# balazs-bamer/cdpr-simulation

Measured on AMD Instinct MI355X. Metric: CDPR sim-steps/sec (whole node), 65 536 parallel 8-cable robots, 1 ms dt, higher is better.
Workload: dtype f32

## Files before the change

### cdpr-simulation_amd/csrc/cdpr_onestep_kernel.hpp

```cpp
#pragma once
#include "cdpr_step_kernel.hpp"

namespace cdpr {

CDPR_DEV void row_to_lds(const float4* src, float4* dst_row) {
  __builtin_amdgcn_global_load_lds((const __attribute__((address_space(1))) void*)src, (__attribute__((address_space(3))) void*)dst_row, 16, 0, 0);
}


template <int NP, bool PR = false>
CDPR_DEV void pid_pairs(const StepArgs& a, int calls, bool is_vel, const v2f (&desired)[NP], const v2f (&actual)[NP], const v2f (&win)[NP][kWin],
                        v2f (&ierr)[NP], v2f (&f)[NP], v2f (&e_new)[NP], float& dbg_p, float& dbg_i, float& dbg_d, bool is_force = false) {
  const PidCoef c = pid_coef<PR>(a, is_vel);
  const bool run = (!PR || calls != 0) && !is_force;
  const bool full = calls >= c.nbuf;
  const float (&wt)[kWin + 2] = a.wrow;
  v2f error[NP], acc[NP];
#pragma unroll
  for (int k = 0; k < NP; ++k) {
    error[k] = desired[k] - actual[k];
    acc[k] = splat(wt[kWin]) * error[k];
  }
#pragma unroll
  for (int j = 0; j < kWin; ++j) {
// ... 260 lines not shown
  }

  if (PERSIST && more) {
    const uint32_t noff = nrr * 16u;
    if (run_pid) {
#pragma unroll
      for (int j = 0; j < kCtrl; ++j)
        row_to_lds(reinterpret_cast<const float4*>(reinterpret_cast<const char*>(a.state + (size_t)(P + j) * st) + noff), &stage[j][0]);
      if (kCmdLds) {
        const float* ncp = a.cmd + (size_t)nrr * N;
#pragma unroll
        for (int g = 0; g < kCmdRows; ++g) row_to_lds(reinterpret_cast<const float4*>(ncp) + g, &stage[kCtrl + g][0]);
      }
    }
  }

  CDPR_STAMP(5);
  v2f applied[NP];
  int td_flag = 0;
  if (TD) {
    v2f df[NP];
#pragma unroll
    for (int k = 0; k < NP; ++k) df[k] = f[k] - splat(a.td_mid);
    float g[6];
    if (FK) {
      jt_times<NP>(jest, df, g);
      normal_solve<NP, false>(jest, 0.f, g);
    } else {
      jt_times<NP>(jac, df, g);
      normal_solve<NP, false>(jac, 0.f, g);
    }
#pragma unroll
    for (int k = 0; k < NP; ++k) {
      v2f t = splat(a.td_mid);
#pragma unroll
      for (int c = 0; c < 6; ++c) t = fma2(g[c], FK ? jest[k][c] : jac[k][c], t);
      const v2f tc = max2(min2(t, splat(a.td_max)), splat(a.td_min));
      td_flag |= (tc.x != t.x) ? 1 : 0;
      if (2 * k + 1 < N) td_flag |= (tc.y != t.y) ? 1 : 0;
      applied[k] = tc;
    }
  } else {
#pragma unroll
    for (int k = 0; k < NP; ++k) applied[k] = f[k];
  }
  if (a.vel_limit > 0.f) {
#pragma unroll
    for (int k = 0; k < NP; ++k) {
      applied[k].x = (qd[k].x > a.vel_limit && applied[k].x > 0.f) || (qd[k].x < -a.vel_limit && applied[k].x < 0.f) ? 0.f : applied[k].x;
      applied[k].y = (qd[k].y > a.vel_limit && applied[k].y > 0.f) || (qd[k].y < -a.vel_limit && applied[k].y < 0.f) ? 0.f : applied[k].y;
    }
  }
  if (a.effort >= 0.f) {
#pragma unroll
    for (int k = 0; k < NP; ++k) applied[k] = max2(min2(applied[k], splat(a.effort)), splat(-a.effort));
  }

  if (a.dbg && live) {
    float* d = a.dbg + (size_t)r * 9;
    if (dbg_wrote) {
      d[0] = dbg_p;
      d[1] = dbg_i;
      d[2] = dbg_d;
      d[3] = desired[0].x;
    }
    d[4] = applied[0].x;
  }
  if (publish && live) {
    store_slot(a.obs, st, 3, woff, make_float4(s.wz, fk_res, (float)fk_it, pack_flags(td_flag, travel_mask<N>(a, q))));
#pragma unroll
    for (int g = 0; g < G; ++g) {
      const int k0 = 2 * g, k1 = (2 * g + 1 < NP) ? 2 * g + 1 : 2 * g;
      const bool has = (2 * g + 1 < NP);
      store_slot(a.obs, st, 4 + 2 * G + g, woff,
                make_float4(applied[k0].x, applied[k0].y, has ? applied[k1].x : 0.f, has ? applied[k1].y : 0.f));
    }
  }

  CDPR_STAMP(6);
  {
    v2f tens[NP];
#pragma unroll
    for (int k = 0; k < NP; ++k) {
      tens[k] = fma2(-a.damping, qd[k], applied[k]);
      if (a.unilateral) tens[k] = max2(tens[k], splat(0.f));
    }
    if (FK) {
      uint32_t again = 0;
      asm volatile("" : "+v"(again));
      v2f len2[NP], l02[NP];
      ik_pairs<N, false>(lds + again, s.px, s.py, s.pz, s.qx, s.qy, s.qz, s.qw, len2, jac, l02);
    }
    float w[6];
    jt_times<NP>(jac, tens, w);
    w[0] = a.fgx - w[0];
    w[1] = a.fgy - w[1];
    w[2] = a.fgz - w[2];
    w[3] = -w[3];
    w[4] = -w[4];
    w[5] = -w[5];
    integrate(a, s, w);
  }
  if (PERSIST && more) {
    constexpr int kDmaOps = kCtrl + kCmdRows;
    static_assert(kDmaOps < 64, "vmcnt is a 6-bit counter");
    if (run_pid)
      __builtin_amdgcn_s_waitcnt(vmcnt_imm(kDmaOps));
    else
      __builtin_amdgcn_s_waitcnt(vmcnt_imm(0));
    asm volatile("" : "+a"(n0), "+a"(n1), "+a"(n2), "+a"(n3), "+a"(n4));
  }
  if (live) {
    CDPR_STORE_STATE(a.state, st, 0, woff, make_float4(s.px, s.py, s.pz, s.qx));
    CDPR_STORE_STATE(a.state, st, 1, woff, make_float4(s.qy, s.qz, s.qw, s.vx));
    CDPR_STORE_STATE(a.state, st, 2, woff, make_float4(s.vy, s.vz, s.wx, s.wy));
    CDPR_STORE_STATE(a.state, st, 3, woff, make_float4(s.wz, fkx, fky, fkz));
    if (FK) CDPR_STORE_STATE(a.state, st, 4, woff, make_float4(fkqx, fkqy, fkqz, fkqw));
  }
  CDPR_STAMP(7);
  if (!(PERSIST && more)) break;
  blk = nblk;
  r = nr;
  rr = nrr;
  live = r < a.batch;
  off = rr * 16u, woff = r * 16u;
  p0 = make_float4(n0.x, n0.y, n0.z, n0.w), p1 = make_float4(n1.x, n1.y, n1.z, n1.w), p2 = make_float4(n2.x, n2.y, n2.z, n2.w);
  p3 = make_float4(n3.x, n3.y, n3.z, n3.w), p4 = make_float4(n4.x, n4.y, n4.z, n4.w);
  staged = run_pid;
  }
}

#ifndef CDPR_CTL_LOAD_DELAY
#define CDPR_CTL_LOAD_DELAY 8
#endif
#ifndef CDPR_SPLIT_PRIO
#define CDPR_SPLIT_PRIO 1
#endif
#ifdef CDPR_STAMPS
#define CDPR_SPLIT_STAMP(i)                                                                                          \
  do {                                                                                                               \
    __builtin_amdgcn_sched_barrier(0);                                                                               \
    if (a.stamps && lane == 0) a.stamps[(size_t)blockIdx.x * 8 + (i)] = __builtin_amdgcn_s_memrealtime();           \
    __builtin_amdgcn_sched_barrier(0);                                                                               \
  } while (0)
#else
#define CDPR_SPLIT_STAMP(i) do { } while (0)
#endif
#if defined(CDPR_STAMPS) && defined(CDPR_STAMPS_ITER)
#define CDPR_CTL_STAMP(i) do { } while (0)
#else
#define CDPR_CTL_STAMP(i) CDPR_SPLIT_STAMP(i)
#endif

template <int N, int XS, int ES, bool RAISED = true>
CDPR_DEV void split_estimator_wave(const StepArgs& a, float* geo, float gval, uint32_t lane, bool live, size_t st, uint32_t off, uint32_t woff,
                                   const float4& p0, const float4& p1, const float4& p3, const v2f* x_force, v2f* x_tension, float* x_est) {
  constexpr int NP = cable_pairs(N);
#if defined(CDPR_STAMPS) && defined(CDPR_STAMPS_CLOCK)
  const unsigned long long clk0 = __builtin_amdgcn_s_memtime();
#endif
#if CDPR_SPLIT_PRIO == 1 || CDPR_SPLIT_PRIO == 4
  if (RAISED) __builtin_amdgcn_s_setprio(3);
#elif CDPR_SPLIT_PRIO == 3 || CDPR_SPLIT_PRIO == 5
  if (RAISED) __builtin_amdgcn_s_setprio(2);
#endif
  const float4 p4 = load_slot(a.state, st, 4, off);
  if (lane < NP * kGeomFloatsPerPair) geo[lane] = gval;
  __builtin_amdgcn_fence(__ATOMIC_RELEASE, "wavefront");
  __builtin_amdgcn_wave_barrier();
  __builtin_amdgcn_fence(__ATOMIC_ACQUIRE, "wavefront");
  float fkx = p3.y, fky = p3.z, fkz = p3.w, fkqx = p4.x, fkqy = p4.y, fkqz = p4.z, fkqw = p4.w;
  v2f len[NP];
  {
    v2f jac[NP][6], l0[NP];
    ik_pairs<N, false>(geo, p0.x, p0.y, p0.z, p0.w, p1.x, p1.y, p1.z, len, jac, l0);
  }
  float fk_res = 0.f;
  int fk_it = 0;
  v2f jest[NP][6];
  {
    v2f elen[NP], unused[NP];
    bool active = true;
    for (int it = 0; it < a.fk_iters; ++it) {
      ik_pairs<N, false>(geo, fkx, fky, fkz, fkqx, fkqy, fkqz, fkqw, elen, jest, unused);
      v2f res[NP];
      v2f rm = splat(0.f);
#pragma unroll
      for (int k = 0; k < NP; ++k) {
        res[k] = len[k] - elen[k];
        rm = max2(rm, abs2(res[k]));
      }
      active = active && !(fmaxf(rm.x, rm.y) < a.fk_tol);
      float g[6];
      jt_times<NP>(jest, res, g);
      normal_solve<NP>(jest, a.fk_lambda, g);
      if (active) {
        fkx += g[0];
        fky += g[1];
        fkz += g[2];
        quat_apply_rotvec(fkqx, fkqy, fkqz, fkqw, g[3], g[4], g[5]);
        ++fk_it;
      }
#ifdef CDPR_STAMPS_ITER
      if (it < 3) {
        asm volatile("" ::"v"(fkqw));
        __builtin_amdgcn_sched_barrier(0);
        if (a.stamps && lane == 0) a.stamps[(size_t)blockIdx.x * 8 + 4 + it] = __builtin_amdgcn_s_memrealtime();
        __builtin_amdgcn_sched_barrier(0);
      }
#endif
    }
    ik_pairs<N, false>(geo, fkx, fky, fkz, fkqx, fkqy, fkqz, fkqw, elen, jest, unused);
    v2f rm = splat(0.f);
#pragma unroll
    for (int k = 0; k < NP; ++k) rm = max2(rm, abs2(len[k] - elen[k]));
    fk_res = fmaxf(rm.x, rm.y);
  }
  if (live) store_slot_aux<CDPR_SPLIT_PLAT_AUX>(a.state, st, 4, woff, make_float4(fkqx, fkqy, fkqz, fkqw));
  CDPR_SPLIT_STAMP(1);
  v2f td_l[6][3];
  float td_invd[6];
  normal_matrix_pk<NP, false>(jest, 0.f, td_l);
  chol_factor_pk(td_l, td_invd);
  __builtin_amdgcn_s_waitcnt(0xC07F);
  __builtin_amdgcn_s_barrier();
  CDPR_SPLIT_STAMP(2);
  __builtin_amdgcn_fence(__ATOMIC_ACQUIRE, "workgroup");
  v2f f[NP], df[NP], t_out[NP];
#pragma unroll
  for (int k = 0; k < NP; ++k) {
    f[k] = x_force[k * XS + lane];
    df[k] = f[k] - splat(a.td_mid);
  }
  int td_flag = 0;
  {
    float g[6];
    jt_times<NP>(jest, df, g);
    chol_apply_pk(td_l, td_invd, g);
#pragma unroll
    for (int k = 0; k < NP; ++k) {
      v2f t = splat(a.td_mid);
#pragma unroll
      for (int c = 0; c < 6; ++c) t = fma2(g[c], jest[k][c], t);
      const v2f tc = max2(min2(t, splat(a.td_max)), splat(a.td_min));
      td_flag |= (tc.x != t.x) ? 1 : 0;
      if (2 * k + 1 < N) td_flag |= (tc.y != t.y) ? 1 : 0;
      t_out[k] = tc;
    }
  }
#pragma unroll
  for (int k = 0; k < NP; ++k) x_tension[k * XS + lane] = t_out[k];
  x_est[0 * ES + lane] = fkx;
  x_est[1 * ES + lane] = fky;
  x_est[2 * ES + lane] = fkz;
  x_est[3 * ES + lane] = fk_res;
  x_est[4 * ES + lane] = (float)fk_it;
  x_est[5 * ES + lane] = (float)td_flag;
  __builtin_amdgcn_fence(__ATOMIC_RELEASE, "workgroup");
  __builtin_amdgcn_s_waitcnt(0xC07F);
  CDPR_SPLIT_STAMP(3);
#if defined(CDPR_STAMPS) && defined(CDPR_STAMPS_CLOCK)
  if (a.stamps && lane == 0) a.stamps[(size_t)blockIdx.x * 8 + 7] = __builtin_amdgcn_s_memtime() - clk0;
#endif
  __builtin_amdgcn_s_barrier();
}

template <int N, bool PR = false>
__global__ __launch_bounds__(128, 2) void cdpr_split_kernel(const StepArgs a) {
  constexpr int NP = cable_pairs(N);
  constexpr int P = plat_slots(true);
  constexpr int G = joint_groups(N);
  constexpr int NH = (NP + 1) / 2;
  __shared__ __attribute__((aligned(16))) float lds[2][NP * kGeomFloatsPerPair];
  __shared__ v2f x_force[NP][64];
  __shared__ v2f x_tension[NP][64];
  __shared__ float x_est[6][64];

  const uint32_t swap = __builtin_popcount(blockIdx.x & a.split_swap) & 1u;
  const uint32_t wave = (threadIdx.x >> 6) ^ swap, lane = threadIdx.x & 63u;
  const uint32_t r = blockIdx.x * 64u + lane;
  const uint32_t rr = (r < a.batch) ? r : (a.batch - 1u);
  const bool live = r < a.batch;
  const size_t st = a.stride;
  const uint32_t off = rr * 16u, woff = r * 16u;
  float* const geo = lds[wave];

  if (wave == 0) CDPR_SPLIT_STAMP(0);
#ifdef CDPR_STAMPS
  if (a.stamps && lane == 0)
    reinterpret_cast<uint32_t*>(&a.stamps[(size_t)blockIdx.x * 8 + 7])[threadIdx.x >> 6] =
        (__builtin_amdgcn_s_getreg((16 - 1) << 11 | 4) & 0xffffu) | ((__builtin_amdgcn_s_getreg((4 - 1) << 11 | 20) & 0xfu) << 16);
#endif
  const float gval = (lane < NP * kGeomFloatsPerPair) ? a.geom[lane] : 0.f;
  const float4 p0 = load_slot(a.state, st, 0, off), p1 = load_slot(a.state, st, 1, off), p2 = load_slot(a.state, st, 2, off),
               p3 = load_slot(a.state, st, 3, off);
  if (wave == 0) {
    split_estimator_wave<N, 64, 64>(a, geo, gval, lane, live, st, off, woff, p0, p1, p3, &x_force[0][0], &x_tension[0][0], &x_est[0][0]);
    return;
  }
#if CDPR_SPLIT_PRIO == 2 || CDPR_SPLIT_PRIO == 5
  __builtin_amdgcn_s_setprio(3);
#endif
#if CDPR_CTL_LOAD_DELAY > 0
  __builtin_amdgcn_s_sleep(CDPR_CTL_LOAD_DELAY);
#endif
  constexpr int kCtrl = 5 * NP + NH;
  float4 wraw[NP][5], hraw[NH];
#pragma unroll
  for (int k = 0; k < NP; ++k) {
#pragma unroll
    for (int m = 0; m < 5; ++m) wraw[k][m] = load_slot(a.state, st, P + 5 * k + m, off);
  }
#pragma unroll
  for (int g = 0; g < NH; ++g) hraw[g] = load_slot(a.state, st, P + 5 * NP + g, off);
  (void)kCtrl;
  v2f desired[NP];
#pragma unroll
  for (int k = 0; k < NP; ++k) desired[k] = splat(0.f);
  const float* cp = a.cmd + (size_t)rr * N;
  if (N % 4 == 0) {
#pragma unroll
    for (int g = 0; g < N / 4; ++g) {
      const float4 v = reinterpret_cast<const float4*>(cp)[g];
      desired[2 * g] = (v2f){v.x, v.y};
      desired[2 * g + 1] = (v2f){v.z, v.w};
    }
  } else {
#pragma unroll
    for (int i = 0; i < N; ++i) {
      if (i & 1)
        desired[i / 2].y = cp[i];
      else
        desired[i / 2].x = cp[i];
    }
  }
  if (lane < NP * kGeomFloatsPerPair) geo[lane] = gval;
  __builtin_amdgcn_fence(__ATOMIC_RELEASE, "wavefront");
  __builtin_amdgcn_wave_barrier();
  __builtin_amdgcn_fence(__ATOMIC_ACQUIRE, "wavefront");

  Platform s;
  s.px = p0.x; s.py = p0.y; s.pz = p0.z; s.qx = p0.w;
  s.qy = p1.x; s.qz = p1.y; s.qw = p1.z; s.vx = p1.w;
  s.vy = p2.x; s.vz = p2.y; s.wx = p2.z; s.wy = p2.w;
  s.wz = p3.x;

  v2f len[NP], q[NP], qd[NP], jac[NP][6];
  {
    v2f l0[NP];
    ik_pairs<N, true>(geo, s.px, s.py, s.pz, s.qx, s.qy, s.qz, s.qw, len, jac, l0);
#pragma unroll
    for (int k = 0; k < NP; ++k) {
      q[k] = l0[k] - len[k];
      qd[k] = -fma2(s.wz, jac[k][5], fma2(s.wy, jac[k][4], fma2(s.wx, jac[k][3],
                    fma2(s.vz, jac[k][2], fma2(s.vy, jac[k][1], splat(s.vx) * jac[k][0])))));
    }
  }
  const bool publish = (a.publish_mask & 1ull) != 0ull;
  if (publish && live) {
    store_slot(a.obs, st, 0, woff, make_float4(s.px, s.py, s.pz, s.qx));
    store_slot(a.obs, st, 1, woff, make_float4(s.qy, s.qz, s.qw, s.vx));
    store_slot(a.obs, st, 2, woff, make_float4(s.vy, s.vz, s.wx, s.wy));
#pragma unroll
    for (int g = 0; g < G; ++g) {
      const int k0 = 2 * g, k1 = (2 * g + 1 < NP) ? 2 * g + 1 : 2 * g;
      const bool has = (2 * g + 1 < NP);
      store_slot(a.obs, st, 4 + g, woff, make_float4(q[k0].x, q[k0].y, has ? q[k1].x : 0.f, has ? q[k1].y : 0.f));
      store_slot(a.obs, st, 4 + G + g, woff, make_float4(qd[k0].x, qd[k0].y, has ? qd[k1].x : 0.f, has ? qd[k1].y : 0.f));
    }
  }

  v2f f[NP], e_new[NP], ierr[NP];
#pragma unroll
  for (int k = 0; k < NP; ++k) {
    f[k] = splat(0.f);
    e_new[k] = splat(0.f);
    ierr[k] = (k & 1) ? (v2f){hraw[k / 2].z, hraw[k / 2].w} : (v2f){hraw[k / 2].x, hraw[k / 2].y};
  }
  float dbg_p = 0.f, dbg_i = 0.f, dbg_d = 0.f;
  bool dbg_wrote = false;
  const bool first_world = (a.flags & kFlagFirstWorldStep) != 0u;
  uint32_t meta = 0u;
  if (PR) meta = a.meta[rr];
  const int calls = PR ? (int)(meta >> kMetaCallShift) : a.pid_calls;
  if (PR && live && !first_world) a.meta[r] = (uint8_t)((meta & kMetaModeMask) | ((uint32_t)min(calls + 1, (int)kMetaCallMax) << kMetaCallShift));
  const bool force_mode = !PR && (a.flags & kFlagForceMode) != 0u;
  if (force_mode && !first_world) {
#pragma unroll
    for (int k = 0; k < NP; ++k) f[k] = desired[k];
  } else if (!first_world && (PR || calls != 0)) {
    v2f win[NP][kWin];
#pragma unroll
    for (int k = 0; k < NP; ++k) {
#pragma unroll
      for (int m = 0; m < 5; ++m) {
        win[k][2 * m] = (v2f){wraw[k][m].x, wraw[k][m].y};
        win[k][2 * m + 1] = (v2f){wraw[k][m].z, wraw[k][m].w};
      }
    }
    const bool actual_is_vel = PR ? ((meta & kMetaModeMask) == kMetaVelocity) : ((a.flags & kFlagActualIsVelocity) != 0u);
    v2f actual[NP];
#pragma unroll
    for (int k = 0; k < NP; ++k) actual[k] = actual_is_vel ? qd[k] : q[k];
    const int ring_slot = a.ring_slot;
    const bool is_force = PR && (meta & kMetaModeMask) == kMetaForce;
#if CDPR_SPLIT_PRIO == 3 || CDPR_SPLIT_PRIO == 4
    __builtin_amdgcn_s_setprio(3);
#endif
    pid_pairs<NP, PR>(a, calls, actual_is_vel, desired, actual, win, ierr, f, e_new, dbg_p, dbg_i, dbg_d, is_force);
    dbg_wrote = (!PR || calls != 0) && !is_force;
    if (live) {
#pragma unroll
      for (int m = 0; m < 5; ++m) {
        if (m == (ring_slot >> 1)) {
#pragma unroll
          for (int k = 0; k < NP; ++k) CDPR_STORE_STATE(a.state, st, P + 5 * k + m, woff, ring_row(win[k], m, e_new[k], ring_slot));
        }
      }
#pragma unroll
      for (int g = 0; g < NH; ++g) {
        const int k1 = (2 * g + 1 < NP) ? 2 * g + 1 : 2 * g;
        CDPR_STORE_STATE(a.state, st, P + 5 * NP + g, woff, make_float4(ierr[2 * g].x, ierr[2 * g].y, ierr[k1].x, ierr[k1].y));
      }
    }
  }
#pragma unroll
  for (int k = 0; k < NP; ++k) x_force[k][lane] = f[k];
  __builtin_amdgcn_fence(__ATOMIC_RELEASE, "workgroup");
  __builtin_amdgcn_s_waitcnt(0xC07F);
  CDPR_CTL_STAMP(4);
#if CDPR_SPLIT_PRIO >= 3
  __builtin_amdgcn_s_setprio(0);
#endif
  __builtin_amdgcn_s_barrier();
  __builtin_amdgcn_s_barrier();
  CDPR_CTL_STAMP(5);
  __builtin_amdgcn_fence(__ATOMIC_ACQUIRE, "workgroup");
  v2f applied[NP];
#pragma unroll
  for (int k = 0; k < NP; ++k) applied[k] = x_tension[k][lane];
  const float fkx = x_est[0][lane], fky = x_est[1][lane], fkz = x_est[2][lane], fk_res = x_est[3][lane], fk_it = x_est[4][lane],
              td_flag = x_est[5][lane];
  if (a.vel_limit > 0.f) {
#pragma unroll
    for (int k = 0; k < NP; ++k) {
      applied[k].x = (qd[k].x > a.vel_limit && applied[k].x > 0.f) || (qd[k].x < -a.vel_limit && applied[k].x < 0.f) ? 0.f : applied[k].x;
      applied[k].y = (qd[k].y > a.vel_limit && applied[k].y > 0.f) || (qd[k].y < -a.vel_limit && applied[k].y < 0.f) ? 0.f : applied[k].y;
    }
  }
  if (a.effort >= 0.f) {
#pragma unroll
    for (int k = 0; k < NP; ++k) applied[k] = max2(min2(applied[k], splat(a.effort)), splat(-a.effort));
  }
  if (a.dbg && live) {
    float* d = a.dbg + (size_t)r * 9;
    if (dbg_wrote) {
      d[0] = dbg_p;
      d[1] = dbg_i;
      d[2] = dbg_d;
      d[3] = desired[0].x;
    }
    d[4] = applied[0].x;
  }
  if (publish && live) {
    store_slot(a.obs, st, 3, woff, make_float4(s.wz, fk_res, fk_it, a.travel_on ? pack_flags((int)td_flag, travel_mask<N>(a, q)) : td_flag));
#pragma unroll
    for (int g = 0; g < G; ++g) {
      const int k0 = 2 * g, k1 = (2 * g + 1 < NP) ? 2 * g + 1 : 2 * g;
      const bool has = (2 * g + 1 < NP);
      store_slot(a.obs, st, 4 + 2 * G + g, woff,
                 make_float4(applied[k0].x, applied[k0].y, has ? applied[k1].x : 0.f, has ? applied[k1].y : 0.f));
    }
  }
  {
    v2f tens[NP];
#pragma unroll
    for (int k = 0; k < NP; ++k) {
      tens[k] = fma2(-a.damping, qd[k], applied[k]);
      if (a.unilateral) tens[k] = max2(tens[k], splat(0.f));
    }
    float w[6];
    jt_times<NP>(jac, tens, w);
    w[0] = a.fgx - w[0];
    w[1] = a.fgy - w[1];
    w[2] = a.fgz - w[2];
    w[3] = -w[3];
    w[4] = -w[4];
    w[5] = -w[5];
    integrate(a, s, w);
  }
  if (live) {
    store_slot_aux<CDPR_SPLIT_PLAT_AUX>(a.state, st, 0, woff, make_float4(s.px, s.py, s.pz, s.qx));
    store_slot_aux<CDPR_SPLIT_PLAT_AUX>(a.state, st, 1, woff, make_float4(s.qy, s.qz, s.qw, s.vx));
    store_slot_aux<CDPR_SPLIT_PLAT_AUX>(a.state, st, 2, woff, make_float4(s.vy, s.vz, s.wx, s.wy));
    store_slot_aux<CDPR_SPLIT_PLAT_AUX>(a.state, st, 3, woff, make_float4(s.wz, fkx, fky, fkz));
  }
  CDPR_CTL_STAMP(6);
}

}
```

### cdpr-simulation_amd/csrc/cdpr_step_kernel.hpp

```cpp
#pragma once
#include <hip/hip_runtime.h>
#include <stdint.h>

namespace cdpr {

constexpr int kMaxCables = 8;
constexpr int kWin = 10;
constexpr int kGeomFloatsPerPair = 16;

typedef float v2f __attribute__((ext_vector_type(2)));

enum StepFlags : uint32_t {
  kFlagFirstWorldStep = 1u << 0,
  kFlagRolloutResetPid = 1u << 1,
  kFlagActualIsVelocity = 1u << 2,
  kFlagPublishAll = 1u << 4,
  kFlagForceMode = 1u << 3,
};

struct PidSet {
  float kf, kp, ki, kd, inv_ki, imax, imin, cmax, cmin;
  int clamp_cmd;
};

// ... 234 lines not shown
    for (int i = j + 1; i < 6; ++i) {
      float s = m[i][j];
#pragma unroll
      for (int k = 0; k < j; ++k) s = fmaf(-m[i][k], m[j][k], s);
      m[i][j] = s * invd[j];
    }
  }
#pragma unroll
  for (int i = 0; i < 6; ++i) {
    float s = g[i];
#pragma unroll
    for (int k = 0; k < i; ++k) s = fmaf(-m[i][k], g[k], s);
    g[i] = s * invd[i];
  }
#pragma unroll
  for (int i = 5; i >= 0; --i) {
    float s = g[i];
#pragma unroll
    for (int k = i + 1; k < 6; ++k) s = fmaf(-m[k][i], g[k], s);
    g[i] = s * invd[i];
  }
}

#ifndef CDPR_CHOL_PACKED
#define CDPR_CHOL_PACKED 1
#endif

CDPR_DEV void chol_factor_pk(v2f (&mp)[6][3], float (&invd)[6]) {
#pragma unroll
  for (int j = 0; j < 6; ++j) {
    const int p0 = j / 2;
    invd[j] = __frsqrt_rn((j & 1) ? mp[j][p0].y : mp[j][p0].x);
#pragma unroll
    for (int p = p0; p < 3; ++p) mp[j][p] = mp[j][p] * splat(invd[j]);
#pragma unroll
    for (int c = j + 1; c < 6; ++c) {
      const float lcj = (c & 1) ? mp[j][c / 2].y : mp[j][c / 2].x;
#pragma unroll
      for (int p = c / 2; p < 3; ++p) mp[c][p] = fma2(-lcj, mp[j][p], mp[c][p]);
    }
  }
}

CDPR_DEV void chol_apply_pk(const v2f (&mp)[6][3], const float (&invd)[6], float (&g)[6]) {
  v2f gp[3] = {(v2f){g[0], g[1]}, (v2f){g[2], g[3]}, (v2f){g[4], g[5]}};
#pragma unroll
  for (int j = 0; j < 6; ++j) {
    g[j] = ((j & 1) ? gp[j / 2].y : gp[j / 2].x) * invd[j];
#pragma unroll
    for (int p = (j + 1) / 2; p < 3; ++p) gp[p] = fma2(-g[j], mp[j][p], gp[p]);
  }
#pragma unroll
  for (int i = 5; i >= 0; --i) {
    float s = g[i];
#pragma unroll
    for (int k = i + 1; k < 6; ++k) s = fmaf(-((k & 1) ? mp[i][k / 2].y : mp[i][k / 2].x), g[k], s);
    g[i] = s * invd[i];
  }
}

CDPR_DEV void chol_solve_pk(v2f (&mp)[6][3], float (&g)[6]) {
  float invd[6];
  chol_factor_pk(mp, invd);
  chol_apply_pk(mp, invd, g);
}

template <int NP, bool LAMBDA = true>
CDPR_DEV void normal_matrix_pk(const v2f (&jac)[NP][6], float lambda, v2f (&mp)[6][3]) {
  v2f acc[21];
  gram_partial<NP>(jac, acc);
#pragma unroll
  for (int a = 0, e = 0; a < 6; ++a) {
#pragma unroll
    for (int b = 0; b <= a; ++b, ++e) {
      const float v = (LAMBDA && a == b) ? hsum(acc[e]) + lambda : hsum(acc[e]);
      if (a & 1)
        mp[b][a / 2].y = v;
      else
        mp[b][a / 2].x = v;
    }
  }
  mp[1][0].x = 0.f;
  mp[3][1].x = 0.f;
  mp[5][2].x = 0.f;
}

template <int NP, bool LAMBDA = true>
CDPR_DEV void normal_solve(const v2f (&jac)[NP][6], float lambda, float (&g)[6]) {
#if CDPR_CHOL_PACKED
  v2f mp[6][3];
  normal_matrix_pk<NP, LAMBDA>(jac, lambda, mp);
  chol_solve_pk(mp, g);
#else
  v2f acc[21];
  gram_partial<NP>(jac, acc);
  float m[6][6];
#pragma unroll
  for (int a = 0, e = 0; a < 6; ++a) {
#pragma unroll
    for (int b = 0; b <= a; ++b, ++e) m[a][b] = (LAMBDA && a == b) ? hsum(acc[e]) + lambda : hsum(acc[e]);
  }
  chol_solve(m, g);
#endif
}

struct PidCoef {
  float kf, kp, ki, kd, inv_ki, imax, imin, cmax, cmin;
  int nbuf;
  bool clamp;
};
template <bool PR>
CDPR_DEV PidCoef pid_coef(const StepArgs& a, bool is_vel) {
  PidCoef c;
  const bool alt = PR && !is_vel;
  c.kf = alt ? a.alt.kf : a.kf;
  c.kp = alt ? a.alt.kp : a.kp;
  c.ki = alt ? a.alt.ki : a.ki;
  c.kd = alt ? a.alt.kd : a.kd;
  c.inv_ki = alt ? a.alt.inv_ki : a.inv_ki;
  c.imax = alt ? a.alt.imax : a.imax;
  c.imin = alt ? a.alt.imin : a.imin;
  c.cmax = alt ? a.alt.cmax : a.cmax;
  c.cmin = alt ? a.alt.cmin : a.cmin;
  c.nbuf = a.nbuf;
  c.clamp = (alt ? a.alt.clamp_cmd : a.clamp_cmd) != 0;
  return c;
}
constexpr uint32_t kMetaModeMask = 3u, kMetaCallShift = 2u, kMetaCallMax = 63u;
constexpr uint32_t kMetaForce = 0u, kMetaPosition = 1u, kMetaVelocity = 2u;

struct Platform {
  float px, py, pz, qx, qy, qz, qw;
  float vx, vy, vz, wx, wy, wz;
};

CDPR_DEV void integrate_pose(const StepArgs& a, Platform& s);
CDPR_DEV void integrate_velocity(const StepArgs& a, Platform& s, const float (&w)[6]) {
  const Rot r = quat_to_rot(s.qx, s.qy, s.qz, s.qw);
  s.vx = fmaf(a.dt_inv_mass, w[0], s.vx);
  s.vy = fmaf(a.dt_inv_mass, w[1], s.vy);
  s.vz = fmaf(a.dt_inv_mass, w[2], s.vz);
  float tbx = fmaf(r.r20, w[5], fmaf(r.r10, w[4], r.r00 * w[3]));
  float tby = fmaf(r.r21, w[5], fmaf(r.r11, w[4], r.r01 * w[3]));
  float tbz = fmaf(r.r22, w[5], fmaf(r.r12, w[4], r.r02 * w[3]));
  const float obx = fmaf(r.r20, s.wz, fmaf(r.r10, s.wy, r.r00 * s.wx));
  const float oby = fmaf(r.r21, s.wz, fmaf(r.r11, s.wy, r.r01 * s.wx));
  const float obz = fmaf(r.r22, s.wz, fmaf(r.r12, s.wy, r.r02 * s.wx));
  const float iox = fmaf(a.ib[4], obz, fmaf(a.ib[3], oby, a.ib[0] * obx));
  const float ioy = fmaf(a.ib[5], obz, fmaf(a.ib[1], oby, a.ib[3] * obx));
  const float ioz = fmaf(a.ib[2], obz, fmaf(a.ib[5], oby, a.ib[4] * obx));
  tbx -= fmaf(oby, ioz, -(obz * ioy));
  tby -= fmaf(obz, iox, -(obx * ioz));
  tbz -= fmaf(obx, ioy, -(oby * iox));
  const float abx = fmaf(a.ibinv[4], tbz, fmaf(a.ibinv[3], tby, a.ibinv[0] * tbx));
  const float aby = fmaf(a.ibinv[5], tbz, fmaf(a.ibinv[1], tby, a.ibinv[3] * tbx));
  const float abz = fmaf(a.ibinv[2], tbz, fmaf(a.ibinv[5], tby, a.ibinv[4] * tbx));
  s.wx = fmaf(a.dt, fmaf(r.r02, abz, fmaf(r.r01, aby, r.r00 * abx)), s.wx);
  s.wy = fmaf(a.dt, fmaf(r.r12, abz, fmaf(r.r11, aby, r.r10 * abx)), s.wy);
  s.wz = fmaf(a.dt, fmaf(r.r22, abz, fmaf(r.r21, aby, r.r20 * abx)), s.wz);
}

CDPR_DEV void integrate_pose(const StepArgs& a, Platform& s) {
  s.px = fmaf(a.dt, s.vx, s.px);
  s.py = fmaf(a.dt, s.vy, s.py);
  s.pz = fmaf(a.dt, s.vz, s.pz);
  const float h = a.half_dt;
  const float nx = fmaf(h, fmaf(-s.wz, s.qy, fmaf(s.wy, s.qz, s.qw * s.wx)), s.qx);
  const float ny = fmaf(h, fmaf(-s.wx, s.qz, fmaf(s.wz, s.qx, s.qw * s.wy)), s.qy);
  const float nz = fmaf(h, fmaf(-s.wy, s.qx, fmaf(s.wx, s.qy, s.qw * s.wz)), s.qz);
  const float nw = fmaf(-h, fmaf(s.wz, s.qz, fmaf(s.wy, s.qy, s.wx * s.qx)), s.qw);
  const float inv = __frsqrt_rn(fmaf(nw, nw, fmaf(nz, nz, fmaf(ny, ny, nx * nx))));
  s.qx = nx * inv;
  s.qy = ny * inv;
  s.qz = nz * inv;
  s.qw = nw * inv;
}

CDPR_DEV void integrate(const StepArgs& a, Platform& s, const float (&w)[6]) {
  integrate_velocity(a, s, w);
  integrate_pose(a, s);
}

template <int N>
CDPR_DEV uint32_t travel_mask(const StepArgs& a, const v2f (&q)[cable_pairs(N)]) {
  uint32_t m = 0u;
  if (a.travel_on) {
#pragma unroll
    for (int k = 0; k < cable_pairs(N); ++k) {
      m |= (q[k].x < a.travel_lo || q[k].x > a.travel_hi) ? (1u << (2 * k)) : 0u;
      if (2 * k + 1 < N) m |= (q[k].y < a.travel_lo || q[k].y > a.travel_hi) ? (1u << (2 * k + 1)) : 0u;
    }
  }
  return m;
}
CDPR_DEV float pack_flags(int td_flag, uint32_t limit_mask) { return (float)((uint32_t)td_flag | (limit_mask << 1)); }

template <int N>
CDPR_DEV void apply_travel_stop(const StepArgs& a, Platform& s, const v2f (&q)[cable_pairs(N)], const v2f (&jac)[cable_pairs(N)][6]) {
  const Rot r = quat_to_rot(s.qx, s.qy, s.qz, s.qw);
  float vx = s.vx, vy = s.vy, vz = s.vz, wx = s.wx, wy = s.wy, wz = s.wz;
  for (int sweep = 0; sweep < a.travel_stop; ++sweep)
#pragma unroll
  for (int i = 0; i < N; ++i) {
    const int k = i / 2;
    float j[6];
#pragma unroll
    for (int c = 0; c < 6; ++c) j[c] = (i & 1) ? jac[k][c].y : jac[k][c].x;
    const float qi = (i & 1) ? q[k].y : q[k].x;
    const float qdn = -fmaf(j[5], wz, fmaf(j[4], wy, fmaf(j[3], wx, fmaf(j[2], vz, fmaf(j[1], vy, j[0] * vx)))));
    const bool hit = (qi >= a.travel_hi && qdn > 0.f) || (qi <= a.travel_lo && qdn < 0.f);
    const float tbx = fmaf(r.r20, j[5], fmaf(r.r10, j[4], r.r00 * j[3]));
    const float tby = fmaf(r.r21, j[5], fmaf(r.r11, j[4], r.r01 * j[3]));
    const float tbz = fmaf(r.r22, j[5], fmaf(r.r12, j[4], r.r02 * j[3]));
    const float abx = fmaf(a.ibinv[4], tbz, fmaf(a.ibinv[3], tby, a.ibinv[0] * tbx));
    const float aby = fmaf(a.ibinv[5], tbz, fmaf(a.ibinv[1], tby, a.ibinv[3] * tbx));
    const float abz = fmaf(a.ibinv[2], tbz, fmaf(a.ibinv[5], tby, a.ibinv[4] * tbx));
    const float awx = fmaf(r.r02, abz, fmaf(r.r01, aby, r.r00 * abx));
    const float awy = fmaf(r.r12, abz, fmaf(r.r11, aby, r.r10 * abx));
    const float awz = fmaf(r.r22, abz, fmaf(r.r21, aby, r.r20 * abx));
    const float d = fmaf(j[5], awz, fmaf(j[4], awy, fmaf(j[3], awx, fmaf(j[2], j[2], fmaf(j[1], j[1], j[0] * j[0])) * a.inv_mass)));
    const float lam = hit ? qdn / d : 0.f;
    const float lm = lam * a.inv_mass;
    vx = fmaf(lm, j[0], vx);
    vy = fmaf(lm, j[1], vy);
    vz = fmaf(lm, j[2], vz);
    wx = fmaf(lam, awx, wx);
    wy = fmaf(lam, awy, wy);
    wz = fmaf(lam, awz, wz);
  }
  s.vx = vx, s.vy = vy, s.vz = vz, s.wx = wx, s.wy = wy, s.wz = wz;
}

template <int N>
CDPR_DEV void integrate_lumped_velocity(const StepArgs& a, const float* lds, Platform& s, const v2f (&jac)[cable_pairs(N)][6],
                                        const v2f (&len)[cable_pairs(N)], float (&w)[6]) {
  constexpr int NP = cable_pairs(N);
  const Rot r = quat_to_rot(s.qx, s.qy, s.qz, s.qw);
  v2f fx = splat(0.f), fy = splat(0.f), fz = splat(0.f), tx = splat(0.f), ty = splat(0.f), tz = splat(0.f);
  v2f sa = splat(0.f), sax = splat(0.f), say = splat(0.f), saz = splat(0.f);
  v2f ixx = splat(0.f), iyy = splat(0.f), izz = splat(0.f), ixy = splat(0.f), ixz = splat(0.f), iyz = splat(0.f);
  v2f gram[21];
#pragma unroll
  for (int e = 0; e < 21; ++e) gram[e] = splat(0.f);
#pragma unroll
  for (int k = 0; k < NP; ++k) {
    const float4 g1 = *reinterpret_cast<const float4*>(lds + k * kGeomFloatsPerPair + 4);
    const float4 g2 = *reinterpret_cast<const float4*>(lds + k * kGeomFloatsPerPair + 8);
    const float4 g3 = *reinterpret_cast<const float4*>(lds + k * kGeomFloatsPerPair + 12);
    const v2f mask = ((N & 1) && k == NP - 1) ? (v2f){g3.z, g3.w} : splat(1.f);
    const v2f bx = {g1.z, g1.w}, by = {g2.x, g2.y}, bz = {g2.z, g2.w};
    const v2f rbx = fma2(r.r02, bz, fma2(r.r01, by, splat(r.r00) * bx));
    const v2f rby = fma2(r.r12, bz, fma2(r.r11, by, splat(r.r10) * bx));
    const v2f rbz = fma2(r.r22, bz, fma2(r.r21, by, splat(r.r20) * bx));
    const v2f ux = jac[k][0], uy = jac[k][1], uz = jac[k][2];
    const v2f l = (mask.x == 0.f || mask.y == 0.f) ? (v2f){len[k].x + (1.f - mask.x), len[k].y + (1.f - mask.y)} : len[k];
    const v2f il = (v2f){__frcp_rn(l.x), __frcp_rn(l.y)};
    const v2f vpx = fma2(s.wy, rbz, fma2(-s.wz, rby, splat(s.vx)));
    const v2f vpy = fma2(s.wz, rbx, fma2(-s.wx, rbz, splat(s.vy)));
    const v2f vpz = fma2(s.wx, rby, fma2(-s.wy, rbx, splat(s.vz)));
    const v2f along = fma2(uz, vpz, fma2(uy, vpy, ux * vpx));
    const v2f vtx = fma2(-along, ux, vpx), vty = fma2(-along, uy, vpy), vtz = fma2(-along, uz, vpz);
    const v2f oux = fma2(s.wy, uz, -(splat(s.wz) * uy)), ouy = fma2(s.wz, ux, -(splat(s.wx) * uz)), ouz = fma2(s.wx, uy, -(splat(s.wy) * ux));
    const v2f uvx = fma2(uy, vpz, -(uz * vpy)), uvy = fma2(uz, vpx, -(ux * vpz)), uvz = fma2(ux, vpy, -(uy * vpx));
    const v2f cl = splat(-a.ph_c) * il * mask;
    const v2f two_il = il + il;
    const v2f fdx = cl * fma2(two_il, vtx, -oux), fdy = cl * fma2(two_il, vty, -ouy), fdz = cl * fma2(two_il, vtz, -ouz);
    const v2f pm = splat(a.ph_mpt) * mask;
    const v2f fax = fma2(a.gx, pm, fdx), fay = fma2(a.gy, pm, fdy), faz = fma2(a.gz, pm, fdz);
    fx += fax;
    fy += fay;
    fz += faz;
    const v2f cm = splat(a.ph_c) * mask;
    tx += fma2(rby, faz, -(rbz * fay)) + cm * fma2(uvx, il, splat(-s.wx));
    ty += fma2(rbz, fax, -(rbx * faz)) + cm * fma2(uvy, il, splat(-s.wy));
    tz += fma2(rbx, fay, -(rby * fax)) + cm * fma2(uvz, il, splat(-s.wz));
    const v2f mu = splat(a.ph_jleg) * il * il;
    const v2f alpha = (mu + splat(a.ph_mpt)) * mask, beta = (splat(a.ph_max) - mu) * mask;
    sa += alpha;
    sax = fma2(alpha, rbx, sax);
    say = fma2(alpha, rby, say);
    saz = fma2(alpha, rbz, saz);
    const v2f rb2 = fma2(rbz, rbz, fma2(rby, rby, rbx * rbx));
    ixx = fma2(alpha, fma2(-rbx, rbx, rb2), ixx);
    iyy = fma2(alpha, fma2(-rby, rby, rb2), iyy);
    izz = fma2(alpha, fma2(-rbz, rbz, rb2), izz);
    ixy = fma2(-alpha, rbx * rby, ixy);
    ixz = fma2(-alpha, rbx * rbz, ixz);
    iyz = fma2(-alpha, rby * rbz, iyz);
    v2f bj[6];
#pragma unroll
    for (int c = 0; c < 6; ++c) bj[c] = beta * jac[k][c];
#pragma unroll
    for (int p = 0, e = 0; p < 6; ++p) {
#pragma unroll
      for (int q = 0; q <= p; ++q, ++e) gram[e] = fma2(bj[p], jac[k][q], gram[e]);
    }
  }
  const float b00 = a.ib[0], b11 = a.ib[1], b22 = a.ib[2], b01 = a.ib[3], b02 = a.ib[4], b12 = a.ib[5];
  const float c00 = fmaf(r.r02, b02, fmaf(r.r01, b01, r.r00 * b00)), c01 = fmaf(r.r02, b12, fmaf(r.r01, b11, r.r00 * b01)), c02 = fmaf(r.r02, b22, fmaf(r.r01, b12, r.r00 * b02));
  const float c10 = fmaf(r.r12, b02, fmaf(r.r11, b01, r.r10 * b00)), c11 = fmaf(r.r12, b12, fmaf(r.r11, b11, r.r10 * b01)), c12 = fmaf(r.r12, b22, fmaf(r.r11, b12, r.r10 * b02));
  const float c20 = fmaf(r.r22, b02, fmaf(r.r21, b01, r.r20 * b00)), c21 = fmaf(r.r22, b12, fmaf(r.r21, b11, r.r20 * b01)), c22 = fmaf(r.r22, b22, fmaf(r.r21, b12, r.r20 * b02));
  const float w00 = fmaf(c02, r.r02, fmaf(c01, r.r01, c00 * r.r00)) + a.ph_iadd_total, w11 = fmaf(c12, r.r12, fmaf(c11, r.r11, c10 * r.r10)) + a.ph_iadd_total,
              w22 = fmaf(c22, r.r22, fmaf(c21, r.r21, c20 * r.r20)) + a.ph_iadd_total;
  const float w01 = fmaf(c02, r.r12, fmaf(c01, r.r11, c00 * r.r10)), w02 = fmaf(c02, r.r22, fmaf(c01, r.r21, c00 * r.r20)),
              w12 = fmaf(c12, r.r22, fmaf(c11, r.r21, c10 * r.r20));
  const float iox = fmaf(w02, s.wz, fmaf(w01, s.wy, w00 * s.wx)), ioy = fmaf(w12, s.wz, fmaf(w11, s.wy, w01 * s.wx)), ioz = fmaf(w22, s.wz, fmaf(w12, s.wy, w02 * s.wx));
// ... 597 lines not shown
```

Baseline: 6.479 billion.

## Move control-wave stores and integrator precompute into estimator wait window

The estimator wave now writes its FK estimate to LDS before the first barrier, so the controller wave can read it sooner. The controller wave moves its observation and PID-ring/integral global stores, plus a tension-independent prelude of the velocity integration (rotation matrix and gyroscopic term) and the travel mask, to the span between the two barriers, where it previously sat idle waiting for the estimator's tension solve. The intent is to fill that idle window and shorten the serial critical path after the tension arrives. The cost is a longer live range for the window registers and PID state, which adds register pressure.

Measured after the change: 6.429 billion. About the same (-0.8%).

```diff
diff --git a/cdpr-simulation_amd/csrc/cdpr_onestep_kernel.hpp b/cdpr-simulation_amd/csrc/cdpr_onestep_kernel.hpp
--- a/cdpr-simulation_amd/csrc/cdpr_onestep_kernel.hpp
+++ b/cdpr-simulation_amd/csrc/cdpr_onestep_kernel.hpp
@@ -436,7 +436,7 @@
 #define CDPR_CTL_STAMP(i) CDPR_SPLIT_STAMP(i)
 #endif
 
-template <int N, int XS, int ES, bool RAISED = true>
+template <int N, int XS, int ES, bool RAISED = true, bool EARLY_EST = false>
 CDPR_DEV void split_estimator_wave(const StepArgs& a, float* geo, float gval, uint32_t lane, bool live, size_t st, uint32_t off, uint32_t woff,
                                    const float4& p0, const float4& p1, const float4& p3, const v2f* x_force, v2f* x_tension, float* x_est) {
   constexpr int NP = cable_pairs(N);
@@ -506,7 +506,16 @@
   float td_invd[6];
   normal_matrix_pk<NP, false>(jest, 0.f, td_l);
   chol_factor_pk(td_l, td_invd);
+  if (EARLY_EST) {
+    x_est[0 * ES + lane] = fkx;
+    x_est[1 * ES + lane] = fky;
+    x_est[2 * ES + lane] = fkz;
+    x_est[3 * ES + lane] = fk_res;
+    x_est[4 * ES + lane] = (float)fk_it;
+    __builtin_amdgcn_fence(__ATOMIC_RELEASE, "workgroup");
+  }
   __builtin_amdgcn_s_waitcnt(0xC07F);
+  __builtin_amdgcn_sched_barrier(0);
   __builtin_amdgcn_s_barrier();
   CDPR_SPLIT_STAMP(2);
   __builtin_amdgcn_fence(__ATOMIC_ACQUIRE, "workgroup");
@@ -534,11 +543,13 @@
   }
 #pragma unroll
   for (int k = 0; k < NP; ++k) x_tension[k * XS + lane] = t_out[k];
-  x_est[0 * ES + lane] = fkx;
-  x_est[1 * ES + lane] = fky;
-  x_est[2 * ES + lane] = fkz;
-  x_est[3 * ES + lane] = fk_res;
-  x_est[4 * ES + lane] = (float)fk_it;
+  if (!EARLY_EST) {
+    x_est[0 * ES + lane] = fkx;
+    x_est[1 * ES + lane] = fky;
+    x_est[2 * ES + lane] = fkz;
+    x_est[3 * ES + lane] = fk_res;
+    x_est[4 * ES + lane] = (float)fk_it;
+  }
   x_est[5 * ES + lane] = (float)td_flag;
   __builtin_amdgcn_fence(__ATOMIC_RELEASE, "workgroup");
   __builtin_amdgcn_s_waitcnt(0xC07F);
@@ -579,7 +590,7 @@
   const float4 p0 = load_slot(a.state, st, 0, off), p1 = load_slot(a.state, st, 1, off), p2 = load_slot(a.state, st, 2, off),
                p3 = load_slot(a.state, st, 3, off);
   if (wave == 0) {
-    split_estimator_wave<N, 64, 64>(a, geo, gval, lane, live, st, off, woff, p0, p1, p3, &x_force[0][0], &x_tension[0][0], &x_est[0][0]);
+    split_estimator_wave<N, 64, 64, true, true>(a, geo, gval, lane, live, st, off, woff, p0, p1, p3, &x_force[0][0], &x_tension[0][0], &x_est[0][0]);
     return;
   }
 #if CDPR_SPLIT_PRIO == 2 || CDPR_SPLIT_PRIO == 5
@@ -641,18 +652,6 @@
     }
   }
   const bool publish = (a.publish_mask & 1ull) != 0ull;
-  if (publish && live) {
-    store_slot(a.obs, st, 0, woff, make_float4(s.px, s.py, s.pz, s.qx));
-    store_slot(a.obs, st, 1, woff, make_float4(s.qy, s.qz, s.qw, s.vx));
-    store_slot(a.obs, st, 2, woff, make_float4(s.vy, s.vz, s.wx, s.wy));
-#pragma unroll
-    for (int g = 0; g < G; ++g) {
-      const int k0 = 2 * g, k1 = (2 * g + 1 < NP) ? 2 * g + 1 : 2 * g;
-      const bool has = (2 * g + 1 < NP);
-      store_slot(a.obs, st, 4 + g, woff, make_float4(q[k0].x, q[k0].y, has ? q[k1].x : 0.f, has ? q[k1].y : 0.f));
-      store_slot(a.obs, st, 4 + G + g, woff, make_float4(qd[k0].x, qd[k0].y, has ? qd[k1].x : 0.f, has ? qd[k1].y : 0.f));
-    }
-  }
 
   v2f f[NP], e_new[NP], ierr[NP];
 #pragma unroll
@@ -669,44 +668,30 @@
   const int calls = PR ? (int)(meta >> kMetaCallShift) : a.pid_calls;
   if (PR && live && !first_world) a.meta[r] = (uint8_t)((meta & kMetaModeMask) | ((uint32_t)min(calls + 1, (int)kMetaCallMax) << kMetaCallShift));
   const bool force_mode = !PR && (a.flags & kFlagForceMode) != 0u;
+  const bool pid_runs = !first_world && !force_mode && (PR || calls != 0);
+  v2f win[NP][kWin];
+#pragma unroll
+  for (int k = 0; k < NP; ++k) {
+#pragma unroll
+    for (int m = 0; m < 5; ++m) {
+      win[k][2 * m] = (v2f){wraw[k][m].x, wraw[k][m].y};
+      win[k][2 * m + 1] = (v2f){wraw[k][m].z, wraw[k][m].w};
+    }
+  }
   if (force_mode && !first_world) {
 #pragma unroll
     for (int k = 0; k < NP; ++k) f[k] = desired[k];
-  } else if (!first_world && (PR || calls != 0)) {
-    v2f win[NP][kWin];
-#pragma unroll
-    for (int k = 0; k < NP; ++k) {
-#pragma unroll
-      for (int m = 0; m < 5; ++m) {
-        win[k][2 * m] = (v2f){wraw[k][m].x, wraw[k][m].y};
-        win[k][2 * m + 1] = (v2f){wraw[k][m].z, wraw[k][m].w};
-      }
-    }
+  } else if (pid_runs) {
     const bool actual_is_vel = PR ? ((meta & kMetaModeMask) == kMetaVelocity) : ((a.flags & kFlagActualIsVelocity) != 0u);
     v2f actual[NP];
 #pragma unroll
     for (int k = 0; k < NP; ++k) actual[k] = actual_is_vel ? qd[k] : q[k];
-    const int ring_slot = a.ring_slot;
     const bool is_force = PR && (meta & kMetaModeMask) == kMetaForce;
 #if CDPR_SPLIT_PRIO == 3 || CDPR_SPLIT_PRIO == 4
     __builtin_amdgcn_s_setprio(3);
 #endif
     pid_pairs<NP, PR>(a, calls, actual_is_vel, desired, actual, win, ierr, f, e_new, dbg_p, dbg_i, dbg_d, is_force);
     dbg_wrote = (!PR || calls != 0) && !is_force;
-    if (live) {
-#pragma unroll
-      for (int m = 0; m < 5; ++m) {
-        if (m == (ring_slot >> 1)) {
-#pragma unroll
-          for (int k = 0; k < NP; ++k) CDPR_STORE_STATE(a.state, st, P + 5 * k + m, woff, ring_row(win[k], m, e_new[k], ring_slot));
-        }
-      }
-#pragma unroll
-      for (int g = 0; g < NH; ++g) {
-        const int k1 = (2 * g + 1 < NP) ? 2 * g + 1 : 2 * g;
-        CDPR_STORE_STATE(a.state, st, P + 5 * NP + g, woff, make_float4(ierr[2 * g].x, ierr[2 * g].y, ierr[k1].x, ierr[k1].y));
-      }
-    }
   }
 #pragma unroll
   for (int k = 0; k < NP; ++k) x_force[k][lane] = f[k];
@@ -717,14 +702,46 @@
   __builtin_amdgcn_s_setprio(0);
 #endif
   __builtin_amdgcn_s_barrier();
+  __builtin_amdgcn_fence(__ATOMIC_ACQUIRE, "workgroup");
+  const float fkx = x_est[0][lane], fky = x_est[1][lane], fkz = x_est[2][lane], fk_res = x_est[3][lane], fk_it = x_est[4][lane];
+  if (publish && live) {
+    store_slot(a.obs, st, 0, woff, make_float4(s.px, s.py, s.pz, s.qx));
+    store_slot(a.obs, st, 1, woff, make_float4(s.qy, s.qz, s.qw, s.vx));
+    store_slot(a.obs, st, 2, woff, make_float4(s.vy, s.vz, s.wx, s.wy));
+#pragma unroll
+    for (int g = 0; g < G; ++g) {
+      const int k0 = 2 * g, k1 = (2 * g + 1 < NP) ? 2 * g + 1 : 2 * g;
+      const bool has = (2 * g + 1 < NP);
+      store_slot(a.obs, st, 4 + g, woff, make_float4(q[k0].x, q[k0].y, has ? q[k1].x : 0.f, has ? q[k1].y : 0.f));
+      store_slot(a.obs, st, 4 + G + g, woff, make_float4(qd[k0].x, qd[k0].y, has ? qd[k1].x : 0.f, has ? qd[k1].y : 0.f));
+    }
+  }
+  if (pid_runs && live) {
+    const int ring_slot = a.ring_slot;
+#pragma unroll
+    for (int m = 0; m < 5; ++m) {
+      if (m == (ring_slot >> 1)) {
+#pragma unroll
+        for (int k = 0; k < NP; ++k) CDPR_STORE_STATE(a.state, st, P + 5 * k + m, woff, ring_row(win[k], m, e_new[k], ring_slot));
+      }
+    }
+#pragma unroll
+    for (int g = 0; g < NH; ++g) {
+      const int k1 = (2 * g + 1 < NP) ? 2 * g + 1 : 2 * g;
+      CDPR_STORE_STATE(a.state, st, P + 5 * NP + g, woff, make_float4(ierr[2 * g].x, ierr[2 * g].y, ierr[k1].x, ierr[k1].y));
+    }
+  }
+  const VelocityPre vpre = integrate_velocity_pre(a, s);
+  const uint32_t tmask = travel_mask<N>(a, q);
+  asm volatile("" ::"v"(vpre.gx), "v"(vpre.gy), "v"(vpre.gz), "v"(vpre.r.r00), "v"(vpre.r.r11), "v"(vpre.r.r22), "v"(tmask));
+  __builtin_amdgcn_sched_barrier(0);
   __builtin_amdgcn_s_barrier();
   CDPR_CTL_STAMP(5);
   __builtin_amdgcn_fence(__ATOMIC_ACQUIRE, "workgroup");
   v2f applied[NP];
 #pragma unroll
   for (int k = 0; k < NP; ++k) applied[k] = x_tension[k][lane];
-  const float fkx = x_est[0][lane], fky = x_est[1][lane], fkz = x_est[2][lane], fk_res = x_est[3][lane], fk_it = x_est[4][lane],
-              td_flag = x_est[5][lane];
+  const float td_flag = x_est[5][lane];
   if (a.vel_limit > 0.f) {
 #pragma unroll
     for (int k = 0; k < NP; ++k) {
@@ -747,7 +764,7 @@
     d[4] = applied[0].x;
   }
   if (publish && live) {
-    store_slot(a.obs, st, 3, woff, make_float4(s.wz, fk_res, fk_it, a.travel_on ? pack_flags((int)td_flag, travel_mask<N>(a, q)) : td_flag));
+    store_slot(a.obs, st, 3, woff, make_float4(s.wz, fk_res, fk_it, a.travel_on ? pack_flags((int)td_flag, tmask) : td_flag));
 #pragma unroll
     for (int g = 0; g < G; ++g) {
       const int k0 = 2 * g, k1 = (2 * g + 1 < NP) ? 2 * g + 1 : 2 * g;
@@ -771,7 +788,8 @@
     w[3] = -w[3];
     w[4] = -w[4];
     w[5] = -w[5];
-    integrate(a, s, w);
+    integrate_velocity_post(a, s, w, vpre);
+    integrate_pose(a, s);
   }
   if (live) {
     store_slot_aux<CDPR_SPLIT_PLAT_AUX>(a.state, st, 0, woff, make_float4(s.px, s.py, s.pz, s.qx));
diff --git a/cdpr-simulation_amd/csrc/cdpr_step_kernel.hpp b/cdpr-simulation_amd/csrc/cdpr_step_kernel.hpp
--- a/cdpr-simulation_amd/csrc/cdpr_step_kernel.hpp
+++ b/cdpr-simulation_amd/csrc/cdpr_step_kernel.hpp
@@ -410,6 +410,44 @@
   tbx -= fmaf(oby, ioz, -(obz * ioy));
   tby -= fmaf(obz, iox, -(obx * ioz));
   tbz -= fmaf(obx, ioy, -(oby * iox));
+  const float abx = fmaf(a.ibinv[4], tbz, fmaf(a.ibinv[3], tby, a.ibinv[0] * tbx));
+  const float aby = fmaf(a.ibinv[5], tbz, fmaf(a.ibinv[1], tby, a.ibinv[3] * tbx));
+  const float abz = fmaf(a.ibinv[2], tbz, fmaf(a.ibinv[5], tby, a.ibinv[4] * tbx));
+  s.wx = fmaf(a.dt, fmaf(r.r02, abz, fmaf(r.r01, aby, r.r00 * abx)), s.wx);
+  s.wy = fmaf(a.dt, fmaf(r.r12, abz, fmaf(r.r11, aby, r.r10 * abx)), s.wy);
+  s.wz = fmaf(a.dt, fmaf(r.r22, abz, fmaf(r.r21, aby, r.r20 * abx)), s.wz);
+}
+
+struct VelocityPre {
+  Rot r;
+  float gx, gy, gz;
+};
+CDPR_DEV VelocityPre integrate_velocity_pre(const StepArgs& a, const Platform& s) {
+  VelocityPre p;
+  p.r = quat_to_rot(s.qx, s.qy, s.qz, s.qw);
+  const Rot& r = p.r;
+  const float obx = fmaf(r.r20, s.wz, fmaf(r.r10, s.wy, r.r00 * s.wx));
+  const float oby = fmaf(r.r21, s.wz, fmaf(r.r11, s.wy, r.r01 * s.wx));
+  const float obz = fmaf(r.r22, s.wz, fmaf(r.r12, s.wy, r.r02 * s.wx));
+  const float iox = fmaf(a.ib[4], obz, fmaf(a.ib[3], oby, a.ib[0] * obx));
+  const float ioy = fmaf(a.ib[5], obz, fmaf(a.ib[1], oby, a.ib[3] * obx));
+  const float ioz = fmaf(a.ib[2], obz, fmaf(a.ib[5], oby, a.ib[4] * obx));
+  p.gx = fmaf(oby, ioz, -(obz * ioy));
+  p.gy = fmaf(obz, iox, -(obx * ioz));
+  p.gz = fmaf(obx, ioy, -(oby * iox));
+  return p;
+}
+CDPR_DEV void integrate_velocity_post(const StepArgs& a, Platform& s, const float (&w)[6], const VelocityPre& p) {
+  const Rot& r = p.r;
+  s.vx = fmaf(a.dt_inv_mass, w[0], s.vx);
+  s.vy = fmaf(a.dt_inv_mass, w[1], s.vy);
+  s.vz = fmaf(a.dt_inv_mass, w[2], s.vz);
+  float tbx = fmaf(r.r20, w[5], fmaf(r.r10, w[4], r.r00 * w[3]));
+  float tby = fmaf(r.r21, w[5], fmaf(r.r11, w[4], r.r01 * w[3]));
+  float tbz = fmaf(r.r22, w[5], fmaf(r.r12, w[4], r.r02 * w[3]));
+  tbx -= p.gx;
+  tby -= p.gy;
+  tbz -= p.gz;
   const float abx = fmaf(a.ibinv[4], tbz, fmaf(a.ibinv[3], tby, a.ibinv[0] * tbx));
   const float aby = fmaf(a.ibinv[5], tbz, fmaf(a.ibinv[1], tby, a.ibinv[3] * tbx));
   const float abz = fmaf(a.ibinv[2], tbz, fmaf(a.ibinv[5], tby, a.ibinv[4] * tbx));
```
